# tyh666/News-Recommendation-MIND

Hardware: AMD Instinct MI355X
Metric: impressions/sec (train) + candidates scored/sec (eval), NRMS MIND-large 1/8 GPU (higher is better)
Workload: dtype f32; 1 GPU; NRMS train step: MHA news encoder + MHA user encoder, H=384, 12 heads, V=30522 word table (trainable), dropout 0.2, Adam; launch=hipGraph replay of the whole step, global_batch=32, per_gpu_batch=32, candidates=5, history=50, seq_len=30, parallelism=dp1

## Files before the change

### news-recommendation-mind_amd/csrc/gemm_fast64.hip

```cpp
#include "gemm_fast_impl.h"

namespace nrfast {

int launch_modes64(const Args& g, const GemmRoute& r, hipStream_t s) {
  return launch_modes<64, 64>(g, r, s);
}

struct PairArgs {
  Args a, b;
  int ga, off, gb;
};

constexpr int pair_max(int x, int y) { return x > y ? x : y; }

template <int BM, int BN, int AM1, int BMODE1, bool TR1, int AM2, int BMODE2, bool TR2>
__global__ __launch_bounds__(256, 2) void gemm_fast_pair_kernel(PairArgs p) {
  using LA1 = Loader<BM, AM1>;
  using LB1 = Loader<BN, BMODE1>;
  using LA2 = Loader<BM, AM2>;
  using LB2 = Loader<BN, BMODE2>;
  __shared__ __attribute__((aligned(16))) float lds[pair_max(2 * (LA1::LDS_FLOATS + LB1::LDS_FLOATS),
                                                             2 * (LA2::LDS_FLOATS + LB2::LDS_FLOATS))];
  static_assert(LA1::LDS_FLOATS % 4 == 0 && LA2::LDS_FLOATS % 4 == 0, "the B images stay 16-B aligned");
  const int b = (int)blockIdx.x;
  if (b < p.off) {
    if (b >= p.ga) return;
    gemm_fast_body<BM, BN, AM1, BMODE1, TR1>(p.a, b, p.ga, reinterpret_cast<float(*)[LA1::LDS_FLOATS]>(lds),
                                             reinterpret_cast<float(*)[LB1::LDS_FLOATS]>(lds + 2 * LA1::LDS_FLOATS));
  } else {
    gemm_fast_body<BM, BN, AM2, BMODE2, TR2>(p.b, b - p.off, p.gb, reinterpret_cast<float(*)[LA2::LDS_FLOATS]>(lds),
                                             reinterpret_cast<float(*)[LB2::LDS_FLOATS]>(lds + 2 * LA2::LDS_FLOATS));
  }
}

int launch_pair64(const Args& a, const Args& b, hipStream_t s) {
  auto kern = gemm_fast_pair_kernel<64, 64, KC_PLAIN, MN_PLAIN, true, MN_PLAIN, MN_PLAIN, false>;
  const int64_t ua = ((a.M + 63) / 64) * ((a.N + 63) / 64) * a.splits;
  const int64_t ub = ((b.M + 63) / 64) * ((b.N + 63) / 64) * b.splits;
  if (ua <= 0 || ub <= 0 || ua > 0x3fffffff || ub > 0x3fffffff) return NR_EINVAL(0);
  PairArgs p;
  p.a = a;
  p.b = b;
  pair_grids(ua, ub, resident_slots<256>(kern), p.ga, p.off, p.gb);
  hipLaunchKernelGGL(kern, dim3((unsigned)(p.off + p.gb)), dim3(256), 0, s, p);
  NR_LAUNCH_CHECK();
  return NR_OK;
}

}
```

### news-recommendation-mind_amd/csrc/gemm_fast_impl.h

```cpp
#pragma once
#include "gemm_fast_common.h"

namespace nrfast {


template <int BM, int BN, int AM, int BMODE, bool TR>
__device__ __forceinline__ void gemm_fast_body(Args g, const int bid, const int G,
                                               float (*As)[Loader<BM, AM>::LDS_FLOATS],
                                               float (*Bs)[Loader<BN, BMODE>::LDS_FLOATS]) {
  using LA = Loader<BM, AM>;
  using LB = Loader<BN, BMODE>;
  constexpr bool IDX_AHEAD = AM == MN_GATHER || BMODE == MN_GATHER;

  clamp_extents(g);
  const int tid = threadIdx.x, lane = tid & 63, w = tid >> 6, h = lane >> 5, c = lane & 31;
  const int gn = (int)((g.N + BN - 1) / BN);
  const int ntiles = (int)((g.M + BM - 1) / BM) * gn;
  const int units = ntiles * g.splits;
#define NR_WALK_PART 1
#include "gemm_walk.h"

  constexpr int TI = BM / 64, TJ = BN / 64;
  const int wm = (w >> 1) * (BM / 2), wn = (w & 1) * (BN / 2);
  f32x16 acc[TI][TJ];
  zero_acc(acc);

  LA la;
  LB lb;
#define NR_WALK_PART 2
#include "gemm_walk.h"
  la.store(As[0], tid);
  lb.store(Bs[0], tid);
  bool staged = step_load();
  __syncthreads();

  bool pending = false;
  int64_t pm0 = 0, pn0 = 0;
  int buf = 0;
  for (;;) {
    if (pending) {
      epilogue_any<TR, TI, TJ>(g, acc, pm0, pn0, wm, wn, h, c);
      zero_acc(acc);
      pending = false;
    }
    const float* a_s = As[buf];
    const float* b_s = Bs[buf];
    const bool had_staged = staged;
#pragma unroll
    for (int q = 0; q < 4; ++q) {
      float4 a[TI], b[TJ];
#pragma unroll
      for (int i = 0; i < TI; ++i) a[i] = la.frag(a_s, wm + 32 * i + c, h, q);
#pragma unroll
      for (int j = 0; j < TJ; ++j) b[j] = lb.frag(b_s, wn + 32 * j + c, h, q);
#pragma unroll
      for (int i = 0; i < TI; ++i)
#pragma unroll
        for (int j = 0; j < TJ; ++j) {
          acc[i][j] = TR ? __builtin_amdgcn_mfma_f32_32x32x2f32(b[j].x, a[i].x, acc[i][j], 0, 0, 0)
                         : __builtin_amdgcn_mfma_f32_32x32x2f32(a[i].x, b[j].x, acc[i][j], 0, 0, 0);
          acc[i][j] = TR ? __builtin_amdgcn_mfma_f32_32x32x2f32(b[j].y, a[i].y, acc[i][j], 0, 0, 0)
                         : __builtin_amdgcn_mfma_f32_32x32x2f32(a[i].y, b[j].y, acc[i][j], 0, 0, 0);
          acc[i][j] = TR ? __builtin_amdgcn_mfma_f32_32x32x2f32(b[j].z, a[i].z, acc[i][j], 0, 0, 0)
                         : __builtin_amdgcn_mfma_f32_32x32x2f32(a[i].z, b[j].z, acc[i][j], 0, 0, 0);
          acc[i][j] = TR ? __builtin_amdgcn_mfma_f32_32x32x2f32(b[j].w, a[i].w, acc[i][j], 0, 0, 0)
                         : __builtin_amdgcn_mfma_f32_32x32x2f32(a[i].w, b[j].w, acc[i][j], 0, 0, 0);
        }
      if (q == 0 && had_staged) {
        la.store(As[buf ^ 1], tid);
        lb.store(Bs[buf ^ 1], tid);
        staged = step_load();
      }
    }
    __syncthreads();
    buf ^= 1;
    const int old = cp.id;
    const int64_t om0 = cp.u.m0, on0 = cp.u.n0;
    if (!had_staged) break;
    advance(cp);
    if (cp.id != old) {
      pending = true;
      pm0 = om0;
      pn0 = on0;
    }
  }
  epilogue_any<TR, TI, TJ>(g, acc, cp.u.m0, cp.u.n0, wm, wn, h, c);
}

template <int BM, int BN, int AM, int BMODE, bool TR>
__global__ __launch_bounds__(256, 2) void gemm_fast_kernel(Args g) {
  __shared__ __attribute__((aligned(16))) float As[2][Loader<BM, AM>::LDS_FLOATS];
  __shared__ __attribute__((aligned(16))) float Bs[2][Loader<BN, BMODE>::LDS_FLOATS];
  gemm_fast_body<BM, BN, AM, BMODE, TR>(g, (int)blockIdx.x, (int)gridDim.x, As, Bs);
}

template <int BM, int BN>
int launch_modes(const Args& g, const GemmRoute& r, hipStream_t s) {
#define NR_KERN(A_, B_, TR_) gemm_fast_kernel<BM, BN, A_, B_, TR_>
#define NR_ROW(A_, B_, TR_) NR_LAUNCH_ROW(256, BM, BN, A_, B_, TR_)
  NR_MODES_KC(NR_ROW) NR_MODES_MN(NR_ROW)
#undef NR_ROW
#undef NR_KERN
  return NR_EINVAL(7);
}

}
```

Baseline: 24700 impressions/s.

## Deepen global-load prefetch pipeline in 64x64 GEMM using register stash stages

```diff
diff --git a/news-recommendation-mind_amd/csrc/gemm_fast64.hip b/news-recommendation-mind_amd/csrc/gemm_fast64.hip
--- a/news-recommendation-mind_amd/csrc/gemm_fast64.hip
+++ b/news-recommendation-mind_amd/csrc/gemm_fast64.hip
@@ -2,8 +2,13 @@
 
 namespace nrfast {
 
+#ifndef NR_FAST64_DEPTH
+#define NR_FAST64_DEPTH 5
+#endif
+constexpr int DEPTH64 = NR_FAST64_DEPTH;
+
 int launch_modes64(const Args& g, const GemmRoute& r, hipStream_t s) {
-  return launch_modes<64, 64>(g, r, s);
+  return launch_modes<64, 64, DEPTH64>(g, r, s);
 }
 
 struct PairArgs {
@@ -25,10 +30,10 @@
   const int b = (int)blockIdx.x;
   if (b < p.off) {
     if (b >= p.ga) return;
-    gemm_fast_body<BM, BN, AM1, BMODE1, TR1>(p.a, b, p.ga, reinterpret_cast<float(*)[LA1::LDS_FLOATS]>(lds),
+    gemm_fast_body<BM, BN, AM1, BMODE1, TR1, DEPTH64>(p.a, b, p.ga, reinterpret_cast<float(*)[LA1::LDS_FLOATS]>(lds),
                                              reinterpret_cast<float(*)[LB1::LDS_FLOATS]>(lds + 2 * LA1::LDS_FLOATS));
   } else {
-    gemm_fast_body<BM, BN, AM2, BMODE2, TR2>(p.b, b - p.off, p.gb, reinterpret_cast<float(*)[LA2::LDS_FLOATS]>(lds),
+    gemm_fast_body<BM, BN, AM2, BMODE2, TR2, DEPTH64>(p.b, b - p.off, p.gb, reinterpret_cast<float(*)[LA2::LDS_FLOATS]>(lds),
                                              reinterpret_cast<float(*)[LB2::LDS_FLOATS]>(lds + 2 * LA2::LDS_FLOATS));
   }
 }
diff --git a/news-recommendation-mind_amd/csrc/gemm_fast_impl.h b/news-recommendation-mind_amd/csrc/gemm_fast_impl.h
--- a/news-recommendation-mind_amd/csrc/gemm_fast_impl.h
+++ b/news-recommendation-mind_amd/csrc/gemm_fast_impl.h
@@ -1,10 +1,16 @@
 #pragma once
+#include <utility>
+
 #include "gemm_fast_common.h"
 
 namespace nrfast {
 
+template <class F, int... S>
+__device__ __forceinline__ bool for_consts(F& f, std::integer_sequence<int, S...>) {
+  return (f(std::integral_constant<int, S>{}) && ...);
+}
 
-template <int BM, int BN, int AM, int BMODE, bool TR>
+template <int BM, int BN, int AM, int BMODE, bool TR, int DEPTH = 2>
 __device__ __forceinline__ void gemm_fast_body(Args g, const int bid, const int G,
                                                float (*As)[Loader<BM, AM>::LDS_FLOATS],
                                                float (*Bs)[Loader<BN, BMODE>::LDS_FLOATS]) {
@@ -42,6 +48,82 @@
       epilogue_any<TR, TI, TJ>(g, acc, pm0, pn0, wm, wn, h, c);
       zero_acc(acc);
       pending = false;
+    }
+    if constexpr (DEPTH > 2) {
+      constexpr int NS = DEPTH - 1;
+      const int left = lp.u.nt - lp.kt;
+      if (staged && lp.id == cp.id && left >= NS && left % NS == 0) {
+        float4 sa[NS][LA::NV], sb[NS][LB::NV];
+        auto stash = [&](int s) __attribute__((always_inline)) {
+#pragma unroll
+          for (int i = 0; i < LA::NV; ++i) sa[s][i] = la.v[i];
+#pragma unroll
+          for (int i = 0; i < LB::NV; ++i) sb[s][i] = lb.v[i];
+        };
+        auto unstash = [&](int s) __attribute__((always_inline)) {
+#pragma unroll
+          for (int i = 0; i < LA::NV; ++i) la.v[i] = sa[s][i];
+#pragma unroll
+          for (int i = 0; i < LB::NV; ++i) lb.v[i] = sb[s][i];
+        };
+        auto quarter = [&](int q) __attribute__((always_inline)) {
+          float4 a[TI], b[TJ];
+#pragma unroll
+          for (int i = 0; i < TI; ++i) a[i] = la.frag(As[buf], wm + 32 * i + c, h, q);
+#pragma unroll
+          for (int j = 0; j < TJ; ++j) b[j] = lb.frag(Bs[buf], wn + 32 * j + c, h, q);
+#pragma unroll
+          for (int i = 0; i < TI; ++i)
+#pragma unroll
+            for (int j = 0; j < TJ; ++j) {
+              acc[i][j] = TR ? __builtin_amdgcn_mfma_f32_32x32x2f32(b[j].x, a[i].x, acc[i][j], 0, 0, 0)
+                             : __builtin_amdgcn_mfma_f32_32x32x2f32(a[i].x, b[j].x, acc[i][j], 0, 0, 0);
+              acc[i][j] = TR ? __builtin_amdgcn_mfma_f32_32x32x2f32(b[j].y, a[i].y, acc[i][j], 0, 0, 0)
+                             : __builtin_amdgcn_mfma_f32_32x32x2f32(a[i].y, b[j].y, acc[i][j], 0, 0, 0);
+              acc[i][j] = TR ? __builtin_amdgcn_mfma_f32_32x32x2f32(b[j].z, a[i].z, acc[i][j], 0, 0, 0)
+                             : __builtin_amdgcn_mfma_f32_32x32x2f32(a[i].z, b[j].z, acc[i][j], 0, 0, 0);
+              acc[i][j] = TR ? __builtin_amdgcn_mfma_f32_32x32x2f32(b[j].w, a[i].w, acc[i][j], 0, 0, 0)
+                             : __builtin_amdgcn_mfma_f32_32x32x2f32(a[i].w, b[j].w, acc[i][j], 0, 0, 0);
+            }
+        };
+        auto next_load = [&](int s) __attribute__((always_inline)) {
+          ++lp.kt;
+          issue(lp);
+          stash(s);
+        };
+        auto step = [&](auto set, auto load) __attribute__((always_inline)) {
+          quarter(0);
+          unstash(decltype(set)::value);
+          la.store(As[buf ^ 1], tid);
+          lb.store(Bs[buf ^ 1], tid);
+          if constexpr (decltype(load)::value) next_load(decltype(set)::value);
+          quarter(1);
+          quarter(2);
+          quarter(3);
+          __syncthreads();
+          buf ^= 1;
+          ++cp.kt;
+        };
+        stash(0);
+        auto fill = [&](auto i) __attribute__((always_inline)) {
+          __builtin_amdgcn_sched_barrier(0);
+          next_load(decltype(i)::value + 1);
+          return true;
+        };
+        for_consts(fill, std::make_integer_sequence<int, NS - 1>{});
+        __builtin_amdgcn_sched_barrier(0);
+        auto round = [&](auto set) __attribute__((always_inline)) {
+          step(set, std::true_type{});
+          return true;
+        };
+        for (int r = left / NS - 1; r > 0; --r) for_consts(round, std::make_integer_sequence<int, NS>{});
+        auto drain = [&](auto set) __attribute__((always_inline)) {
+          step(set, std::false_type{});
+          return true;
+        };
+        for_consts(drain, std::make_integer_sequence<int, NS - 1>{});
+        unstash(NS - 1);
+      }
     }
     const float* a_s = As[buf];
     const float* b_s = Bs[buf];
@@ -87,16 +169,16 @@
   epilogue_any<TR, TI, TJ>(g, acc, cp.u.m0, cp.u.n0, wm, wn, h, c);
 }
 
-template <int BM, int BN, int AM, int BMODE, bool TR>
+template <int BM, int BN, int AM, int BMODE, bool TR, int DEPTH = 2>
 __global__ __launch_bounds__(256, 2) void gemm_fast_kernel(Args g) {
   __shared__ __attribute__((aligned(16))) float As[2][Loader<BM, AM>::LDS_FLOATS];
   __shared__ __attribute__((aligned(16))) float Bs[2][Loader<BN, BMODE>::LDS_FLOATS];
-  gemm_fast_body<BM, BN, AM, BMODE, TR>(g, (int)blockIdx.x, (int)gridDim.x, As, Bs);
+  gemm_fast_body<BM, BN, AM, BMODE, TR, DEPTH>(g, (int)blockIdx.x, (int)gridDim.x, As, Bs);
 }
 
-template <int BM, int BN>
+template <int BM, int BN, int DEPTH = 2>
 int launch_modes(const Args& g, const GemmRoute& r, hipStream_t s) {
-#define NR_KERN(A_, B_, TR_) gemm_fast_kernel<BM, BN, A_, B_, TR_>
+#define NR_KERN(A_, B_, TR_) gemm_fast_kernel<BM, BN, A_, B_, TR_, DEPTH>
 #define NR_ROW(A_, B_, TR_) NR_LAUNCH_ROW(256, BM, BN, A_, B_, TR_)
   NR_MODES_KC(NR_ROW) NR_MODES_MN(NR_ROW)
 #undef NR_ROW
```

Measured after the change: 24790 impressions/s (median of 4 runs). Within noise of the previous version (+0.4%).
